# springmeyer/cov-tiles

Hardware: AMD Instinct MI355X
Metric: GB/s raw COVT bytes decoded + Mvertices/s, z2–z14 tile batch, 1/2/4/8 GPU (higher is better)
Workload: dtype int32

## Files before the change

cov-tiles_amd/__init__.py:

```python
from __future__ import annotations

import ctypes as C
import os
import subprocess
from dataclasses import dataclass
from typing import List, NamedTuple, Optional

import numpy as np

_HERE = os.path.dirname(os.path.abspath(__file__))
_LIB = os.path.join(_HERE, os.environ.get("COVT_LIB_VARIANT", "libcovt.so"))

OK = 0
ERR_UNSUPPORTED_ENCODING = -1
ERR_TRUNCATED = -2
ERR_COUNT_MISMATCH = -3
ERR_BAD_HEADER = -4
ERR_DEVICE = -5
ERR_INVALID_ARG = -6
INPUT_PADDING = 4096
FORMAT_GENC, FORMAT_GEND = 0, 1
FAMILY_RLE, FAMILY_VARINT, FAMILY_FASTPFOR, FAMILY_LANE, FAMILY_SPLIT, FAMILY_SPLIT_FPF, FAMILY_SPLIT_RLE = range(7)
NUM_FAMILIES = 7
DESC_LANE, DESC_SPLIT, DESC_SPLIT_PAD, DESC_SPLIT_FPF = 0x1, 0x2, 0x4, 0x8
# ... 1142 lines not shown

    def feature(self, i: int) -> bytes:
        if not 0 <= i < len(self):
            raise IndexError(i)
        return bytes(self.data[int(self.offsets[i]):int(self.offsets[i + 1])])


@dataclass
class BboxColumn:
    xmin: np.ndarray
    ymin: np.ndarray
    xmax: np.ndarray
    ymax: np.ndarray
    extent: np.ndarray
    n_empty: int = 0

    def __len__(self) -> int:
        return int(self.xmin.size)

    def as_struct(self) -> np.ndarray:
        return np.stack([self.xmin, self.ymin, self.xmax, self.ymax], axis=1)


@dataclass
class MeasuresColumn:
    area: np.ndarray
    length: np.ndarray
    num_coords: np.ndarray

    def __len__(self) -> int:
        return int(self.area.size)


@dataclass
class PropertyColumn:
    name: str
    type: int
    n_features: int
    validity: np.ndarray
    values: np.ndarray
    dict_offsets: Optional[np.ndarray]
    dict_bytes: Optional[np.ndarray]
    n_valid: int

    def valid(self, i: int) -> bool:
        return bool((int(self.validity[i >> 3]) >> (i & 7)) & 1)

    def value(self, i: int):
        if not self.valid(i):
            return None
        if self.type == PROP_BOOLEAN:
            return bool((int(self.values[i >> 3]) >> (i & 7)) & 1)
        if self.type == PROP_INT64:
            return int(self.values[i])
        if self.type == PROP_FLOAT:
            return float(self.values[i])
        k = int(self.values[i])
        return bytes(self.dict_bytes[self.dict_offsets[k]:self.dict_offsets[k + 1]]).decode("utf-8")

    def to_list(self):
        return [self.value(i) for i in range(self.n_features)]


@dataclass
class LayerColumns:
    layer: int
    ids: Optional[np.ndarray]
    geometry: GeometryColumn
    num_bits: int = 0
    column_type: int = 0
    properties: Optional[dict] = None
    wkb: Optional[WkbColumn] = None
    bbox: Optional[BboxColumn] = None
    crs: int = CRS_TILE
    measures: Optional["MeasuresColumn"] = None


_GEOM_FIELD = {GEOMETRY_TYPES: "geometryTypes", GEOMETRY_OFFSETS: "geometryOffsets", PART_OFFSETS: "partOffsets",
               RING_OFFSETS: "ringOffsets", VERTEX_OFFSETS: "vertexOffsets", VERTEX_BUFFER: "vertexBuffer"}


def split_layers(plan: Plan, out: np.ndarray, res: np.ndarray, tile: int = 0) -> List[LayerColumns]:
    layers = {}
    for i in np.nonzero(plan.streams["tile"] == tile)[0]:
        s = plan.streams[i]
        _raise(int(res[i][0]), "stream %d (layer %d, type %d)" % (i, s["layer"], s["stream_type"]))
        if int(s["column_kind"]) == 2:
            continue
        lc = layers.setdefault(int(s["layer"]), LayerColumns(int(s["layer"]), None, GeometryColumn()))
        arr = plan.stream_array(out, int(i))
        if int(s["column_kind"]) == 0:
            lc.ids = arr
        else:
            setattr(lc.geometry, _GEOM_FIELD[int(s["stream_type"])], arr)
            lc.num_bits = int(s["num_bits"])
            lc.column_type = int(s["column_type"])
    return [layers[k] for k in sorted(layers)]


class CovtParser:
    @staticmethod
    def decode_covt(covt_buffer: bytes, fmt: int = FORMAT_GENC, id_mode: int = ID_FORMAT,
                    properties: bool = False, tile_id=None, crs: int = CRS_TILE) -> List[LayerColumns]:
        if crs != CRS_TILE and tile_id is None:
            raise IllegalArgumentException("a CRS other than CRS_TILE needs the tile's (z, x, y)")
        geo = (crs, [tile_id]) if crs != CRS_TILE else (None, None)
        plan = Plan.from_tiles([covt_buffer], fmt, id_mode, PLAN_PROPERTIES if properties else 0)
        _raise(int(plan.tile_status[0]), "decodeLayerMetadata")
        out, res = plan.decode_host()
        layers = split_layers(plan, out, res, 0)
        for lc in layers:
            lc.crs = crs
        if plan.num_geometry_columns:
            wbuf, wres = plan.wkb_host(*geo)
            by_layer = {lc.layer: lc for lc in layers}
            for c in range(plan.num_geometry_columns):
                lc = by_layer.get(int(plan.wkb["layer"][c]))
                if lc is not None and int(wres["status"][c]) == OK:
                    lc.wkb = plan.wkb_column(wbuf, wres, c)
            bbuf, bres = plan.bbox_host(*geo)
            for c in range(plan.num_geometry_columns):
                lc = by_layer.get(int(plan.bbox["layer"][c]))
                if lc is not None and int(bres["status"][c]) == OK:
                    lc.bbox = plan.bbox_column(bbuf, bres, c)
            mbuf, mres = plan.measures_host()
            for c in range(plan.num_geometry_columns):
                lc = by_layer.get(int(plan.measures["layer"][c]))
                if lc is not None and int(mres["status"][c]) == OK:
                    lc.measures = plan.measures_column(mbuf, mres, c)
        if properties and plan.num_property_columns:
            buf, pres = plan.properties_host()
            by_layer = {lc.layer: lc for lc in layers}
            for c in range(plan.num_property_columns):
                L = int(plan.props["layer"][c])
                lc = by_layer.setdefault(L, LayerColumns(L, None, GeometryColumn()))
                if lc.properties is None:
                    lc.properties = {}
                col = plan.property_column(buf, pres, c)
                lc.properties[col.name] = col
            layers = [by_layer[k] for k in sorted(by_layer)]
        return layers


def version() -> str:
    return lib().covt_version().decode()


_BUILD_SOURCES = (
    ("csrc/covt_decode.hip", "csrc/covt_assemble.hip", "csrc/covt_props.hip", "csrc/covt_plan_device.hip",
     "csrc/covt_wkb.hip", "csrc/covt_bbox.hip", "csrc/covt_measures.hip", "csrc/covt_host.cpp")
    + ("../include/covt.h", "csrc/covt_internal.h", "csrc/covt_wave.h", "csrc/covt_segscan.h", "csrc/covt_walk.h",
       "csrc/covt_props_plan.h",
       "csrc/covt_scratch.h", "csrc/covt_coop.h", "csrc/covt_wkb_plan.h", "csrc/covt_bbox_plan.h",
       "csrc/covt_measures_plan.h", "csrc/covt_geo_plan.h", "csrc/covt_arena.h", "csrc/covt_split_plan.h"))


def source_build_id() -> str:
    import hashlib

    h = hashlib.sha256()
    for f in _BUILD_SOURCES:
        with open(os.path.join(_HERE, f), "rb") as fh:
            h.update(fh.read())
    return h.hexdigest()[:16]


def library_build_id() -> str:
    v = version()
    return v.rsplit("src:", 1)[1] if "src:" in v else "unknown"
```

cov-tiles_amd/csrc/covt_decode.hip:

```cpp
#include <hip/hip_runtime.h>
#include <stdint.h>

#include "covt.h"
#include "covt_internal.h"
#include "covt_wave.h"
#include "covt_walk.h"

namespace covt {

constexpr int kWin = 1024;

#ifndef COVT_LONG_STREAM
#define COVT_LONG_STREAM 16384
#endif
#ifndef COVT_LONG_PRIO
#define COVT_LONG_PRIO 2
#endif
#ifndef COVT_RLE_SHORT_SPAN
#define COVT_RLE_SHORT_SPAN 448
#endif
#ifndef COVT_CHUNK_PRIO
#define COVT_CHUNK_PRIO 2
#endif
constexpr int kLongStream = COVT_LONG_STREAM;
#ifdef COVT_TIMING
constexpr int kPhases = 8;
__device__ uint32_t* covt_phase_buf;
__device__ const covt_stream_desc* covt_phase_desc0;
#endif

typedef __attribute__((address_space(3))) const uint16_t lds_cu16;

struct __attribute__((aligned(16))) WaveSmem {
    int32_t misc[4];
    uint16_t cpre[64];
    uint16_t cmask[64];
    union alignas(16) {
        struct {
            uint32_t win[kWin / 4 + 4];
            uint16_t list[kWin];
            uint16_t next[kWin + 8];
            uint16_t grec[64];
        } v;
        struct {
            union {
                uint32_t stage[324];
                uint32_t ring[512];
            };
            uint32_t patch[256];
            uint32_t cbuf[260];
            union {
                uint8_t posx[2][192];
                uint32_t xw[224];
            };
        } f;
    } u;
};
constexpr int kSmemHdr = 272;
constexpr int kFamSmemRle = kSmemHdr + (kWin / 4 + 4) * 4 + kWin * 2 + (kWin + 8) * 2 + 64 * 2;
constexpr int kFamSmemVarint = kSmemHdr + (kWin / 4 + 4) * 4 + kWin * 2;
constexpr int kFamSmemFpf = kSmemHdr + (512 + 256 + 260 + 224) * 4 > kFamSmemVarint
                                ? kSmemHdr + (512 + 256 + 260 + 224) * 4
                                : kFamSmemVarint;
constexpr int kFpfXw = 224;
static_assert(kFamSmemFpf >= kSmemHdr + (int)sizeof(((WaveSmem*)nullptr)->u.f), "FastPFOR scratch stride");
static_assert(kFamSmemVarint >= kSmemHdr + (int)sizeof(((WaveSmem*)nullptr)->u.v.win) +
                                    (int)sizeof(((WaveSmem*)nullptr)->u.v.list), "varint scratch stride");
static_assert(__builtin_offsetof(WaveSmem, u) == kSmemHdr, "WaveSmem header size");
static_assert(kFamSmemRle == (int)sizeof(WaveSmem), "RLE uses the whole scratch");
static_assert(kFamSmemRle % 16 == 0 && kFamSmemVarint % 16 == 0 && kFamSmemFpf % 16 == 0, "16-B strides");

typedef uint32_t u32x4 __attribute__((ext_vector_type(4)));
typedef __attribute__((address_space(1))) const uint32_t g_u32;
typedef __attribute__((address_space(1))) const u32x4 g_v4;
__device__ __forceinline__ const g_u32* g32(uintptr_t a) { return (const g_u32*)a; }
__device__ __forceinline__ uint4 ld128(uintptr_t a16) {
    const u32x4 v = *(const g_v4*)a16;
    return make_uint4(v.x, v.y, v.z, v.w);
}
typedef __attribute__((address_space(1))) const uint8_t g_u8;
__device__ __forceinline__ uint4 ld128_off(const g_u8* base, uint32_t off) {
    const u32x4 v = *(const g_v4*)(base + off);
    return make_uint4(v.x, v.y, v.z, v.w);
}

__device__ __forceinline__ uint32_t ld_le32(const uint8_t* p) {
    const uintptr_t a = (uintptr_t)p;
    const g_u32* q = g32(a & ~(uintptr_t)3);
    return __builtin_amdgcn_alignbyte(q[1], q[0], (uint32_t)(a & 3));
}
__device__ __forceinline__ uint32_t ld_be32(const uint8_t* p) { return __builtin_bswap32(ld_le32(p)); }
__host__ __device__ constexpr uint32_t be_sel(uint32_t sh) {
    return (sh + 3u) | ((sh + 2u) << 8) | ((sh + 1u) << 16) | (sh << 24);
}
__device__ __forceinline__ uint32_t be_word(uint32_t hi, uint32_t lo, uint32_t sel) {
    return __builtin_amdgcn_perm(hi, lo, sel);
}
typedef __attribute__((address_space(4))) const uint32_t c_u32;
typedef __attribute__((address_space(4))) const u32x4 c_v4;
__device__ __forceinline__ uint32_t sld_le32(const uint8_t* p) {
    const uintptr_t a = (uintptr_t)p;
    const c_u32* q = (const c_u32*)(a & ~(uintptr_t)3);
    const uint64_t v = ((uint64_t)q[1] << 32) | q[0];
    return (uint32_t)(v >> (8u * (uint32_t)(a & 3u)));
}
__device__ __forceinline__ uint32_t sld_be32(const uint8_t* p) { return uniu(__builtin_bswap32(sld_le32(p))); }
__device__ __forceinline__ uint4 sld128(uintptr_t a16) {
    const u32x4 v = *(const c_v4*)a16;
    return make_uint4(v.x, v.y, v.z, v.w);
}

__device__ __forceinline__ uint32_t hibits4(uint32_t x) {
    x &= 0x80808080u;
    return ((x >> 7) & 1u) | ((x >> 14) & 2u) | ((x >> 21) & 4u) | ((x >> 28) & 8u);
}
__device__ __forceinline__ uint32_t hibits16(uint4 d) {
    return hibits4(d.x) | (hibits4(d.y) << 4) | (hibits4(d.z) << 8) | (hibits4(d.w) << 12);
}
__device__ __forceinline__ uint32_t range16(int32_t s, int32_t e) {
    s = s < 0 ? 0 : (s > 16 ? 16 : s);
    e = e < 0 ? 0 : (e > 16 ? 16 : e);
    if (e <= s) return 0u;
    return ((1u << e) - 1u) & ~((1u << s) - 1u);
}
typedef unsigned short u16x2 __attribute__((ext_vector_type(2)));
__device__ __forceinline__ uint32_t pext7(uint32_t x) {
    x &= 0x7f7f7f7fu;
    const uint32_t y = __builtin_bit_cast(uint32_t, __builtin_bit_cast(u16x2, x) >> (u16x2){1, 1});
    const uint32_t t = (x & 0x007f007fu) | (y & ~0x007f007fu);
    return (t & 0x3fffu) | ((t >> 2) & ~0x3fffu);
}
__device__ __forceinline__ uint32_t bytemask(int n) {
    return n >= 4 ? 0xffffffffu : (n <= 0 ? 0u : ((1u << (8 * n)) - 1u));
}
__device__ __forceinline__ int32_t zz32(uint32_t e) { return (int32_t)((e >> 1) ^ (0u - (e & 1u))); }
__device__ __forceinline__ int64_t zz64(uint64_t e) { return (int64_t)((e >> 1) ^ (0ull - (e & 1ull))); }

__host__ __device__ __forceinline__ void morton_xy(int32_t code, int nb, uint32_t& x, uint32_t& y) {
    uint32_t v = (uint32_t)code, t;
    t = (v ^ (v >> 1)) & 0x22222222u; v ^= t ^ (t << 1);
    t = (v ^ (v >> 2)) & 0x0c0c0c0cu; v ^= t ^ (t << 2);
    t = (v ^ (v >> 4)) & 0x00f000f0u; v ^= t ^ (t << 4);
    t = (v ^ (v >> 8)) & 0x0000ff00u; v ^= t ^ (t << 8);
    const uint32_t low = nb >= 16 ? 0xffffu : (nb <= 0 ? 0u : ((1u << nb) - 1u));
    const uint32_t top = nb <= 16 ? 0u : ((nb >= 32 ? 0xffffffffu : ((1u << nb) - 1u)) & ~0xffffu);
    const uint32_t hi = code < 0 ? top : 0u;
    x = (v & low) | hi;
    y = ((v >> 16) & low) | hi;
}
__device__ __forceinline__ int32_t morton_half(int nb) {
    const int32_t te = (int32_t)(2u << ((uint32_t)(nb - 2) & 31u));
    return te / 2;
}

struct Carry {
    uint32_t x, y;
};

typedef int32_t i32x4 __attribute__((ext_vector_type(4)));
// ... 1276 lines not shown
            COVT_PHASE(c, 0);
            const int32_t nblocks_page = uni(thissize / kFpfBlock);
            const int32_t jb0 = v0 > done ? min((v0 - done) / kFpfBlock, nblocks_page) : 0;
            const int32_t nblocks = v1 <= done ? 0 : uni(min(nblocks_page, (int32_t)(((int64_t)v1 - done + kFpfBlock - 1) / kFpfBlock)));
            const int32_t nw32 = (int32_t)nw;
            const int32_t bclen = uni((int32_t)(bcw * 4));
            const uint8_t* cb8 = (const uint8_t*)sm.u.f.cbuf;
            int32_t cbase = (int32_t)(4 * (mw0 - bc));
            auto chunk_load = [&](int32_t at) {
                cbase = (int32_t)(4 * (load_words(sm.u.f.cbuf, bc + (at >> 2)) - bc));
            };
            auto walk = [&](int32_t cur, FpfHdr& h) -> int32_t {
                cur = uni(cur);
                cbase = uni(cbase);
                if (!xin && (uint32_t)(cur - cbase) > (uint32_t)(1020 - 260)) chunk_load(cur);
                const int32_t j = cur - cbase;
                const uint32_t hw =
                    uniu(__builtin_amdgcn_alignbyte(sm.u.f.cbuf[(j >> 2) + 1], sm.u.f.cbuf[j >> 2], (uint32_t)j & 3u));
                const int32_t b = (int32_t)(int8_t)(hw & 0xffu);
                const int32_t ce = (int32_t)((hw >> 8) & 0xffu);
                const int32_t hasx = ce > 0 ? 1 : 0;
                const int32_t idx = hasx ? (int32_t)(int8_t)((hw >> 16) & 0xffu) - b : 1;
                const int32_t k = (uint32_t)(idx - 2) <= 30u ? idx : 0;
                const int32_t xsz = __builtin_amdgcn_readlane(xz_v, k);
                const int32_t xc = __builtin_amdgcn_readlane(xc_v, k);
                h.b = b;
                h.ce = ce;
                h.idx = idx;
                h.xcur = (uint32_t)xc;
                h.bcoff = cur + 2 + hasx;
                h.next = h.bcoff + ce;
                xc_v += l == k ? ce : 0;
                const int32_t worst = max(max(max(b - 32, -b), h.next - bclen), max(max(idx - 32, 1 - idx), xc + ce - xsz));
                return worst > 0 ? COVT_ERR_BAD_HEADER : COVT_OK;
            };
            auto xword = [&](int32_t k, uint32_t xs, uint32_t i, uint32_t& xbit) -> int32_t {
                const uint32_t bit = __umul24(i & 31u, (uint32_t)k);
                xbit = bit & 31u;
                return (int32_t)(xs + __umul24(i >> 5, (uint32_t)k) + (bit >> 5));
            };
            auto prefetch = [&](const FpfHdr& hv, int32_t pkv, FpfPre& pr, int slot, bool raw = true) {
                FpfHdr h;
                h.idx = uni(hv.idx);
                h.ce = uni(hv.ce);
                h.xcur = uniu(hv.xcur);
                h.bcoff = uni(hv.bcoff);
                const int32_t pk = uni(pkv);
                if (raw) {
                    const uintptr_t a16 = ((uintptr_t)c.sb + 4u * (uint32_t)pk) & ~(uintptr_t)15;
                    const uint32_t lraw = min((uint32_t)l, 2u * (uint32_t)uni(hv.b) + 1u);
                    pr.raw = ld128_off((const g_u8*)a16, 16u * lraw);
                }
                const int32_t k = h.idx;
                const uint32_t xs = k >= 2 ? (uint32_t)__builtin_amdgcn_readlane(xs_v, k) : 0u;
                uint32_t xb;
                const int32_t wx = xword(k >= 2 ? k : 2, xs, h.xcur + (uint32_t)l, xb);
                const uint32_t xon = (uint32_t)(k >= 2) & (uint32_t)(l < h.ce) & (uint32_t)(wx < nw32);
                if (!xin) {
                    const uint32_t wi = (uint32_t)wx & (0u - xon);
                    const u32x3 xv = *(const g_v3*)((const g_u8*)(((uintptr_t)c.sb) & ~(uintptr_t)3) + 4u * wi);
                    pr.x0 = xv.x;
                    pr.x1 = xv.y;
                    pr.x2 = xv.z;
                }
                const int32_t pb = h.bcoff - cbase;
                pr.pos = cb8[min(pb + l, 4 * 260 - 1)];
                if (h.ce > 64) {
#pragma unroll
                    for (int q = 1; q < 4; ++q)
                        sm.u.f.posx[slot][64 * (q - 1) + l] = cb8[min(pb + l + 64 * q, 4 * 260 - 1)];
                }
            };
            FpfHdr h;
            int32_t pk = (int32_t)p0 + 1;
            int32_t cur0 = 0;
            if (jb0 > 0 && jb0 < nblocks && !c.err) {
                if (skip && skip->done == done) {
                    cur0 = skip->cur0;
                    pk = skip->pk;
                    xc_v = skip->xc;
                } else {
                    int32_t cur = 0, pkk = pk;
                    for (int32_t j = 0; j < jb0; ++j) {
                        if (!xin && (uint32_t)(cur - cbase) > (uint32_t)(1020 - 8)) chunk_load(cur);
                        const int32_t jj = cur - cbase;
                        const uint32_t hw = uniu(__builtin_amdgcn_alignbyte(sm.u.f.cbuf[(jj >> 2) + 1],
                                                                            sm.u.f.cbuf[jj >> 2], (uint32_t)jj & 3u));
                        const int32_t b = (int32_t)(int8_t)(hw & 0xffu);
                        const int32_t ce = (int32_t)((hw >> 8) & 0xffu);
                        const int32_t idx = (int32_t)(int8_t)((hw >> 16) & 0xffu) - b;
                        pkk += 8 * b;
                        xc_v += (ce > 0 && idx >= 2 && idx <= 32 && l == idx) ? ce : 0;
                        cur += ce > 0 ? 3 + ce : 2;
                        if (cur > bclen) { c.err = COVT_ERR_BAD_HEADER; break; }
                    }
                    cur0 = uni(cur);
                    pk = uni(pkk);
                    if (skip) {
                        skip->done = done;
                        skip->cur0 = cur0;
                        skip->pk = pk;
                        skip->xc = xc_v;
                    }
                }
                COVT_PHASE(c, 0);
            }
            auto block = [&](int32_t j, const FpfPre& pc, FpfPre& pn, int slot) {
                FpfHdr hc;
                hc.b = uni(h.b);
                hc.ce = uni(h.ce);
                hc.idx = uni(h.idx);
                hc.xcur = uniu(h.xcur);
                hc.bcoff = uni(h.bcoff);
                hc.next = uni(h.next);
                const int32_t pkc = uni(pk);
                const int32_t b = hc.b;
                const uint32_t o = (sbmis + 4u * (uint32_t)pkc) & 15u;
                const int32_t qoff = (int32_t)(o >> 2);
                {
                    uint4 raw2 = make_uint4(0, 0, 0, 0);
                    if (b == 32) {
                        const uintptr_t a16 = ((uintptr_t)c.sb + 4u * (uint32_t)pkc) & ~(uintptr_t)15;
                        raw2 = sld128(a16 + 1024);
                    }
                    const uint32_t nxt = lane_next(pc.raw.x, raw2.x);
                    uint4 wv;
                    wv.x = be_word(pc.raw.y, pc.raw.x, bsel);
                    wv.y = be_word(pc.raw.z, pc.raw.y, bsel);
                    wv.z = be_word(pc.raw.w, pc.raw.z, bsel);
                    wv.w = be_word(nxt, pc.raw.w, bsel);
                    ((uint4*)sm.u.f.stage)[l] = wv;
                    if (b == 32 && l == 0) {
                        uint4 w2;
                        w2.x = be_word(raw2.y, raw2.x, bsel);
                        w2.y = be_word(raw2.z, raw2.y, bsel);
                        w2.z = be_word(raw2.w, raw2.z, bsel);
                        w2.w = be_word(0u, raw2.w, bsel);
                        ((uint4*)sm.u.f.stage)[64] = w2;
                    }
                }
                if (hc.ce > 0) ((uint4*)sm.u.f.patch)[l] = make_uint4(0, 0, 0, 0);
                wave_sync();
                COVT_PHASE(c, 1);
                if (j + 1 < nblocks) {
                    c.err = walk(hc.next, h);
                    pk = pkc + 8 * b;
                    if (!c.err && pk + 8 * h.b > nw32) c.err = COVT_ERR_TRUNCATED;
                    if (c.err) return;
                }
                prefetch(h, pk, pn, slot ^ 1);
                COVT_PHASE(c, 2);
                uint32_t v[4];
                {
                    const uint32_t mask = b == 32 ? 0xffffffffu : ((1u << b) - 1u);
                    uint32_t bit = __umul24((uint32_t)(l & 7) * 4u, (uint32_t)b);
                    const int32_t wb = (int32_t)__umul24((uint32_t)(l >> 3), (uint32_t)b) + qoff;
#pragma unroll
                    for (int k = 0; k < 4; ++k) {
                        const int32_t wi = wb + (int32_t)(bit >> 5);
                        const uint32_t lo = sm.u.f.stage[wi], hi = sm.u.f.stage[wi + 1];
                        v[k] = __builtin_amdgcn_alignbit(hi, lo, bit & 31u) & mask;
                        bit += (uint32_t)b;
                    }
                }
                COVT_PHASE(c, 3);
#if defined(COVT_ABL_NOEXC)
                if (false) {
#else
                if (hc.ce > 0) {
#endif
                    const int32_t k = hc.idx;
                    const uint32_t xs = k >= 2 ? (uint32_t)__builtin_amdgcn_readlane(xs_v, k) : 0u;
                    const bool el = l < hc.ce;
                    uint32_t ex = 1u;
                    if (k != 1) {
                        uint32_t xbit;
                        const int32_t wi = xword(k, xs, hc.xcur + (uint32_t)l, xbit);
                        uint32_t lo, hi;
                        if (xin) {
                            const int32_t m = el ? wi - (int32_t)mw0 : 0;
                            lo = sm.u.f.cbuf[m];
                            hi = sm.u.f.cbuf[m + 1];
                        } else {
                            lo = wi < nw32 ? be_word(pc.x1, pc.x0, bsel) : 0u;
                            hi = wi + 1 < nw32 ? be_word(pc.x2, pc.x1, bsel) : 0u;
                        }
                        const uint32_t m = k == 32 ? 0xffffffffu : ((1u << k) - 1u);
                        ex = __builtin_amdgcn_alignbit(hi, lo, xbit) & m;
                    }
                    atomicOr(&sm.u.f.patch[el ? pc.pos : (uint32_t)(4 * l)], el ? ex << (b & 31) : 0u);
                    if (hc.ce > 64) {
                        for (int q = 1; q < 4; ++q) {
                            const int32_t e = l + 64 * q;
                            if (e < hc.ce) {
                                const uint32_t ex = k == 1 ? 1u : xget(W, xs, k, hc.xcur + (uint32_t)e);
                                atomicOr(&sm.u.f.patch[sm.u.f.posx[slot][64 * (q - 1) + l]], ex << (b & 31));
                            }
                        }
                    }
                    wave_sync();
                    const uint4 pt = ((const uint4*)sm.u.f.patch)[l];
                    v[0] |= pt.x;
                    v[1] |= pt.y;
                    v[2] |= pt.z;
                    v[3] |= pt.w;
                }
                COVT_PHASE(c, 4);
#if defined(COVT_ABL_NOSTORE)
                sink_values<OP, 4>(v, 0, 0, kFpfBlock, c.nb, c.out, cr);
#else
                if (sum_only)
                    sum_values<OP, 4>(v, (int64_t)done + (int64_t)j * kFpfBlock, kFpfBlock, ax, ay);
                else
                    sink_values<OP, 4>(v, (int64_t)done + (int64_t)j * kFpfBlock, 0, kFpfBlock, c.nb, c.out, cr);
#endif
                wave_sync();
                COVT_PHASE(c, 5);
            };
            FpfPre preB;
            if (jb0 < nblocks && !c.err) {
                c.err = walk(cur0, h);
                if (!c.err && pk + 8 * h.b > nw32) c.err = COVT_ERR_TRUNCATED;
                if (!c.err) {
                    prefetch(h, pk, pre, 0, !spec);
                    if (!sum_only) fpf_prime_stores<OP>(c.out, (int64_t)done + (int64_t)jb0 * kFpfBlock);
                    int32_t j = jb0;
                    do {
                        block(j, pre, preB, 0);
                        if (j + 1 < nblocks && !c.err) block(j + 1, preB, pre, 1);
                        j += 2;
                    } while (j < nblocks && !c.err);
                }
            }
            done += thissize;
            p = ie;
            if (done >= v1) break;
        }
        decoded = L;
        if (!c.err && has_end && p < nw) {
            int32_t vpos = (int32_t)(4 * p);
            const int32_t base = L;
            Win w;
            w.valid = false;
            const bool tail_in = L > 0 && ((int64_t)(vpos & ~15) >> 2) >= mw0 && nw - mw0 <= 255;
            const int32_t got = varint_take<MODE_WORDREV, VAL_VB>(
                sm, c.sb, w, vpos, (int32_t)(4 * nw), c.n - L, true, c.err,
                [&](const uint32_t (&lo)[1], const uint32_t (&hi)[1], int32_t vb, int32_t, int32_t count) {
                    if (sum_only) sum_values<OP, 1>(lo, (int64_t)base + vb, count, ax, ay);
                    else sink_values<OP, 1>(lo, (int64_t)base + vb, 0, count, c.nb, c.out, cr);
                },
                0, nullptr, 0, tail_in ? sm.u.f.cbuf : nullptr, (int32_t)mw0);
            decoded = L + got;
        }
    }
    if (!c.err && has_end) {
        for (int32_t b = decoded; !sum_only && b < c.n; b += 64) {
            uint32_t vv[1] = {0};
            sink_values<OP, 1>(vv, b, 0, c.n - b < 64 ? c.n - b : 64, c.nb, c.out, cr);
        }
        if (OP == COVT_OP_FPF_ZZ_DELTA_XY && (c.n & 1)) c.err = COVT_ERR_COUNT_MISMATCH;
    }
    COVT_PHASE(c, 7);
    c.consumed = c.byte_length;
    if (sum_only) {
        sums->x = lane_bcast(incl_scan(ax), 63);
        sums->y = lane_bcast(incl_scan(ay), 63);
    }
    if (fin) *fin = cr;
}

template <int OP>
__device__ __forceinline__ void run_fastpfor_stream(Ctx& c) {
    WaveSmem& sm = *c.sm;
    const int l = lane_id();
    const Words W{c.sb, c.byte_length / 4};
    const int32_t nw32 = W.nw;
    const uint32_t bsel = be_sel((uint32_t)((uintptr_t)c.sb & 3u));
    Carry cr{0u, 0u};
    int32_t decoded = 0;
    int32_t L = 0;
    int32_t p = 1;
    int xs_v = 0, xz_v = -1, xc_v = 0;
    int32_t mw0 = 0;
    if (c.byte_length > c.avail) { c.err = COVT_ERR_TRUNCATED; }
    if (!c.err && nw32 > 0) {
        const uint32_t head0 = W.uniform(0), head1 = W.uniform(1);
        L = (int32_t)head0;
        if (L < 0) c.err = COVT_ERR_BAD_HEADER;
        L -= L % kFpfBlock;
        if (!c.err && L > c.n) c.err = COVT_ERR_COUNT_MISMATCH;
        int32_t done = 0;
        const uintptr_t s_end = (uintptr_t)c.sb + 4u * (uint32_t)nw32;
        struct WordsRaw {
            uint4 r;
            int32_t base;
            uint32_t sh;
        };
        auto words_issue = [&](int32_t w) -> WordsRaw {
            const uintptr_t addr = (uintptr_t)c.sb + 4u * (uint32_t)w;
            const uintptr_t a16 = addr & ~(uintptr_t)15;
            const uint32_t o = (uint32_t)(addr & 15u);
            const uint32_t lmax = s_end > a16 ? (uint32_t)((s_end - 1 - a16) >> 4) : 0u;
            WordsRaw q;
            q.r = ld128_off((const g_u8*)a16, 16u * min((uint32_t)l, lmax));
            q.base = uni(w - (int32_t)(o >> 2));
            q.sh = o & 3u;
            return q;
        };
        auto words_store = [&](uint32_t* dst, const WordsRaw& q) -> int32_t {
            const uint32_t nx = lane_next(q.r.x);
            const uint32_t sel = be_sel(q.sh);
            const int32_t wl = q.base + 4 * l;
            uint4 wv;
            wv.x = wl < nw32 ? be_word(q.r.y, q.r.x, sel) : 0u;
            wv.y = wl + 1 < nw32 ? be_word(q.r.z, q.r.y, sel) : 0u;
            wv.z = wl + 2 < nw32 ? be_word(q.r.w, q.r.z, sel) : 0u;
            wv.w = wl + 3 < nw32 ? be_word(nx, q.r.w, sel) : 0u;
            wave_sync();
            ((uint4*)dst)[l] = wv;
            wave_sync();
            return q.base;
        };
        auto load_words = [&](uint32_t* dst, int32_t w) -> int32_t { return words_store(dst, words_issue(w)); };
        while (!c.err && done < L) {
            done = uni(done);
            const int32_t thissize = uni((L - done) < kFpfPage ? (L - done) : kFpfPage);
            const int32_t p0 = uni(p);
            if (p0 >= nw32) { c.err = COVT_ERR_TRUNCATED; break; }
            const int64_t ie0 = (int64_t)p0 + (int32_t)(p0 == 1 ? head1 : W.uniform(p0));
            if (ie0 < 0 || ie0 >= nw32) { c.err = COVT_ERR_TRUNCATED; break; }
            int32_t ie = (int32_t)ie0;
            const WordsRaw mq = words_issue(ie);
            const uintptr_t pa = (uintptr_t)c.sb + 4u * (uint32_t)(p0 + 1);
            const uintptr_t A0 = pa & ~(uintptr_t)127;
            const uint32_t glast = s_end > A0 ? (uint32_t)((s_end - 1 - A0) & ~(uintptr_t)15) : 0u;
            const int32_t wbase = uni((int32_t)(p0 + 1) - (int32_t)((pa - A0) >> 2));
            uint4 R = ld128_off((const g_u8*)A0, min(16u * (uint32_t)l, glast));
            int32_t kst = 0;
            int32_t vend = wbase;
            uint32_t prev63 = 0u;
            mw0 = words_store(sm.u.f.cbuf, mq);
            auto mword = [&](int32_t w) -> uint32_t { return uniu(sm.u.f.cbuf[w - mw0]); };
            const int32_t bytesize = (int32_t)mword(ie++);
            if (bytesize < 0 || bytesize > kFpfBcCap) { c.err = COVT_ERR_BAD_HEADER; break; }
            xc_v = 0;
            const int32_t bcw = (bytesize + 3) / 4;
            const int32_t bc = ie;
            if (bc + bcw >= nw32) { c.err = COVT_ERR_TRUNCATED; break; }
            ie += bcw;
            int64_t ie64 = ie;
            {
                int32_t dbase = INT32_MIN / 2;
                auto dword = [&](int32_t w) -> uint32_t {
                    if (w >= mw0 && w < mw0 + 255) return mword(w);
                    if (w < dbase || w >= dbase + 255) dbase = load_words(sm.u.f.ring, w);
                    return uniu(sm.u.f.ring[w - dbase]);
                };
                uint32_t bm = dword((int32_t)ie64++) & ~1u;
                xs_v = 0;
                xz_v = -1;
                while (bm) {
                    const int32_t k = __builtin_ctz(bm) + 1;
                    bm &= bm - 1;
                    if (ie64 >= nw32) { c.err = COVT_ERR_TRUNCATED; break; }
                    const int32_t size = (int32_t)dword((int32_t)ie64++);
                    if (size < 0) { c.err = COVT_ERR_BAD_HEADER; break; }
                    const int64_t groups = ((int64_t)size + 31) / 32;
                    xs_v = l == k ? (int)(uint32_t)ie64 : xs_v;
                    xz_v = l == k ? size : xz_v;
                    ie64 += groups * k;
                    ie64 -= ((groups * 32 - size) * k) / 32;
                }
                if (c.err) break;
            }
            const bool xin = ie64 - mw0 <= 255;
            ie = (int32_t)(ie64 < nw32 ? ie64 : (int64_t)nw32);
            COVT_PHASE(c, 0);
            const int32_t nblocks = uni(thissize / kFpfBlock);
            const int32_t bclen = uni((int32_t)(bcw * 4));
            const uint8_t* cb8 = (const uint8_t*)sm.u.f.cbuf;
            const g_u8* cbyte = (const g_u8*)(c.sb + 4u * (uint32_t)bc);
            int32_t cbase = (int32_t)(4 * (mw0 - bc));
            auto chunk_load = [&](int32_t at) {
                cbase = (int32_t)(4 * (load_words(sm.u.f.cbuf, bc + (at >> 2)) - bc));
            };
            bool fin = false;
            int32_t bneed = INT32_MAX;
            auto stage = [&]() {
                const int32_t k = uni(kst);
                const uint32_t nx = lane_next(R.x, 0u);
                const int32_t w0 = wbase + 256 * k + 4 * l;
                uint4 wv;
                wv.x = w0 < nw32 ? be_word(R.y, R.x, bsel) : 0u;
                wv.y = w0 + 1 < nw32 ? be_word(R.z, R.y, bsel) : 0u;
                wv.z = w0 + 2 < nw32 ? be_word(R.w, R.z, bsel) : 0u;
                wv.w = w0 + 3 < nw32 ? be_word(nx, R.w, bsel) : 0u;
                const int32_t fw = wbase + 256 * k - 1;
                const uint32_t fix = fw < nw32 ? be_word(lane_bcast(R.x, 0), prev63, bsel) : 0u;
                prev63 = lane_bcast(R.w, 63);
                const uint32_t ri = (uint32_t)(256 * k + 4 * l) & 511u;
                wave_sync();
                if (l < 63) {
                    *(uint4*)&sm.u.f.ring[ri] = wv;
                } else {
                    sm.u.f.ring[ri] = wv.x;
                    sm.u.f.ring[ri + 1] = wv.y;
                    sm.u.f.ring[ri + 2] = wv.z;
                }
                if (l == 0 && k > 0) sm.u.f.ring[(uint32_t)(256 * k - 1) & 511u] = fix;
                wave_sync();
                kst = k + 1;
                vend = wbase + 256 * (k + 1) - 1;
                if (!fin || vend < bneed)
                    R = ld128_off((const g_u8*)A0, min(1024u * (uint32_t)(k + 1) + 16u * (uint32_t)l, glast));
                wave_sync();
            };
            int32_t cur = 0, pk = (int32_t)p0 + 1;
            for (int32_t jbat = 0, nbat = 0; jbat < nblocks && !c.err; jbat += nbat) {
                jbat = uni(jbat);
                nbat = uni(min(64, nblocks - jbat));
                uint32_t hw_v = 0u;
                int32_t cur_v = bclen + 1;
                cur = uni(cur);
                cbase = uni(cbase);
                if (!xin && cur <= bclen && (uint32_t)(cur - cbase) > (uint32_t)(1020 - 258)) chunk_load(cur);
                for (int32_t g = 0; g < nbat; ++g) {
                    cur = uni(cur);
                    cbase = uni(cbase);
                    if (cur > bclen) break;
                    if (!xin && cur - cbase > 1020 - 8) {
                        nbat = g;
                        break;
                    }
                    const int32_t q = cur - cbase;
                    const uint32_t hw =
                        uniu(__builtin_amdgcn_alignbyte(sm.u.f.cbuf[(q >> 2) + 1], sm.u.f.cbuf[q >> 2], (uint32_t)q & 3u));
                    const int32_t ce = (int32_t)((hw >> 8) & 0xffu);
                    const int32_t nx = cur + (ce > 0 ? 3 + ce : 2);
                    if (!xin && g > 0 && nx - cbase > 1020) {
                        nbat = g;
                        break;
                    }
                    hw_v = l == g ? hw : hw_v;
                    cur_v = l == g ? cur : cur_v;
                    cur = nx;
                }
                nbat = uni(nbat);
                if (nbat == 0) {
                    c.err = COVT_ERR_BAD_HEADER;
                    break;
                }
                COVT_PHASE(c, 1);
                const bool in = l < nbat;
                const int32_t b_v = (int32_t)(int8_t)(hw_v & 0xffu);
                const int32_t ce_v = (int32_t)((hw_v >> 8) & 0xffu);
                const bool hasx = ce_v > 0;
                const int32_t idx_v = hasx ? (int32_t)(int8_t)((hw_v >> 16) & 0xffu) - b_v : 1;
                const bool arr_k = hasx && idx_v >= 2 && idx_v <= 32;
                const bool arr = in && arr_k;
                int32_t xcur_v = 0;
                for (uint64_t todo = __ballot(arr); todo;) {
                    const int32_t kk = __builtin_amdgcn_readlane(idx_v, (int32_t)__builtin_ctzll(todo));
                    const bool mine = arr && idx_v == kk;
                    const uint32_t v = mine ? (uint32_t)ce_v : 0u;
                    const uint32_t s = incl_scan(v);
                    const int32_t base = __builtin_amdgcn_readlane(xc_v, kk);
                    xcur_v = mine ? base + (int32_t)(s - v) : xcur_v;
                    xc_v += l == kk ? (int32_t)lane_bcast(s, 63) : 0;
                    todo &= ~__ballot(mine);
                }
                const uint32_t w8 = in ? 8u * (uint32_t)(b_v & 63) : 0u;
                const uint32_t pinc = incl_scan(w8);
                const int32_t pk_v = pk + (int32_t)(pinc - w8);
                pk += (int32_t)lane_bcast(pinc, 63);
                int32_t nok = nbat;
                int32_t ferr = 0;
                {
                    const int32_t xsz = lane_get(xz_v, arr_k ? idx_v : 0);
                    bool bad = (uint32_t)b_v > 32u || cur_v + 2 > bclen;
                    bad |= hasx && (cur_v + 3 + ce_v > bclen || (idx_v != 1 && !arr_k));
                    bad |= arr_k && (xsz < 0 || xcur_v + ce_v > xsz);
                    const bool trunc = pk_v + 8 * b_v > nw32;
                    const uint64_t fail = __ballot(in && (bad || trunc));
                    if (fail) {
                        nok = (int32_t)__builtin_ctzll(fail);
                        ferr = __builtin_amdgcn_readlane(bad ? COVT_ERR_BAD_HEADER : COVT_ERR_TRUNCATED, nok);
                    }
                }
                COVT_PHASE(c, 2);
                fin = jbat + nbat >= nblocks || ferr != 0;
                bneed = nok > 0 ? uni(__builtin_amdgcn_readlane(pk_v + 8 * b_v, nok - 1)) : 0;
                if (jbat == 0) stage();
                struct Hdr {
                    int32_t b, ce, idx, pk, bcoff, xo;
                    uint32_t xcur;
                };
                int32_t xo_v = 255;
                if (!xin) {
                    const bool ab = arr && l < nok;
                    const int32_t k = ab ? idx_v : 2;
                    const uint32_t xs = (uint32_t)lane_get(xs_v, k);
                    const uint32_t b0 = __umul24((uint32_t)xcur_v, (uint32_t)k);
                    const uint32_t b1 = __umul24((uint32_t)(xcur_v + ce_v), (uint32_t)k);
                    const int32_t wlo = (int32_t)(xs + (b0 >> 5));
                    const int32_t wn = ab ? (int32_t)((b1 + 31u) >> 5) - (int32_t)(b0 >> 5) + 1 : 0;
                    const uint32_t winc = incl_scan((uint32_t)wn);
                    const int32_t wo = (int32_t)(winc - (uint32_t)wn);
                    const int32_t wend = (int32_t)winc;
                    xo_v = ab && wend <= kFpfXw ? wo : 255;
                    const int32_t tot = uni(min((int32_t)lane_bcast(winc, 63), kFpfXw));
                    const g_u8* sb4 = (const g_u8*)(((uintptr_t)c.sb) & ~(uintptr_t)3);
                    u32x2 d[4];
                    bool okw[4];
#pragma unroll
                    for (int r = 0; r < 4; ++r) {
                        const int32_t t = 64 * r + l;
                        int32_t lo = 0, hi = 64;
#pragma unroll
                        for (int s2 = 0; s2 < 7; ++s2) {
                            const int32_t mid = (lo + hi) >> 1;
                            const bool le = lane_get(wend, mid & 63) <= t;
                            const bool act = lo < hi;
                            lo = act && le ? mid + 1 : lo;
                            hi = act && !le ? mid : hi;
                        }
                        const int32_t g = min(lo, 63);
                        const int32_t w = lane_get(wlo, g) + (t - lane_get(wo, g));
                        okw[r] = t < tot && w < nw32;
                        d[r] = *(const g_v2*)(sb4 + 4u * (okw[r] ? (uint32_t)w : 0u));
                    }
#pragma unroll
                    for (int r = 0; r < 4; ++r)
                        if (64 * r + l < kFpfXw) sm.u.f.xw[64 * r + l] = okw[r] ? be_word(d[r].y, d[r].x, bsel) : 0u;
                    wave_sync();
                }
                const uint32_t f_v = (uint32_t)(b_v & 0xff) | ((uint32_t)ce_v << 8) | ((uint32_t)(idx_v & 0xff) << 16) |
                                     ((uint32_t)xo_v << 24);
                const int32_t bo_v = cur_v + (hasx ? 3 : 2);
                auto rec = [&](int32_t g, Hdr& h) {
                    const uint32_t f = uniu((uint32_t)__builtin_amdgcn_readlane((int32_t)f_v, g));
                    h.b = (int32_t)(f & 0xffu);
                    h.ce = (int32_t)((f >> 8) & 0xffu);
                    h.idx = (int32_t)(int8_t)((f >> 16) & 0xffu);
                    h.xo = (int32_t)(f >> 24);
                    h.xcur = uniu((uint32_t)__builtin_amdgcn_readlane(xcur_v, g));
                    h.bcoff = uni(__builtin_amdgcn_readlane(bo_v, g));
                    h.pk = uni(__builtin_amdgcn_readlane(pk_v, g));
                };
                fpf_prime_stores<OP>(c.out, (int64_t)done + (int64_t)jbat * kFpfBlock);
                auto block = [&](int32_t g) {
                    Hdr hc;
                    rec(g, hc);
                    const int32_t b = hc.b;
                    if (uni(vend) < hc.pk + 8 * b) stage();
                    if (hc.ce > 0) ((uint4*)sm.u.f.patch)[l] = make_uint4(0, 0, 0, 0);
                    COVT_PHASE(c, 3);
                    uint32_t v[4];
                    {
                        const uint32_t mask = b == 32 ? 0xffffffffu : ((1u << b) - 1u);
                        uint32_t bit = __umul24((uint32_t)(l & 7) * 4u, (uint32_t)b);
                        const int32_t r0 = (hc.pk - wbase) & 511;
                        const int32_t wb = (int32_t)__umul24((uint32_t)(l >> 3), (uint32_t)b) + r0;
                        if (r0 + 8 * b <= 511) {
#pragma unroll
                            for (int k = 0; k < 4; ++k) {
                                const int32_t wi = wb + (int32_t)(bit >> 5);
                                const uint32_t lo = sm.u.f.ring[wi], hi = sm.u.f.ring[wi + 1];
                                v[k] = __builtin_amdgcn_alignbit(hi, lo, bit & 31u) & mask;
                                bit += (uint32_t)b;
                            }
                        } else {
#pragma unroll
                            for (int k = 0; k < 4; ++k) {
                                const int32_t wi = wb + (int32_t)(bit >> 5);
                                const uint32_t lo = sm.u.f.ring[wi & 511], hi = sm.u.f.ring[(wi + 1) & 511];
                                v[k] = __builtin_amdgcn_alignbit(hi, lo, bit & 31u) & mask;
                                bit += (uint32_t)b;
                            }
                        }
                    }
                    COVT_PHASE(c, 4);
                    if (hc.ce > 0) {
                        const int32_t k = hc.idx;
                        const bool el = l < hc.ce;
                        const uint32_t pos = cb8[min(max(hc.bcoff - cbase + l, 0), 4 * 260 - 1)];
                        uint32_t ex = 1u;
                        if (k != 1) {
                            const uint32_t xs = (uint32_t)__builtin_amdgcn_readlane(xs_v, k);
                            const uint32_t bb = __umul24(hc.xcur + (uint32_t)l, (uint32_t)k);
                            const uint32_t xbit = bb & 31u;
                            uint32_t lo, hi;
                            if (xin) {
                                const int32_t m = el ? (int32_t)(xs + (bb >> 5)) - mw0 : 0;
                                lo = sm.u.f.cbuf[m];
                                hi = sm.u.f.cbuf[m + 1];
                            } else if (hc.xo != 255) {
                                const int32_t m = el ? hc.xo + (int32_t)(bb >> 5) - (int32_t)(__umul24(hc.xcur, (uint32_t)k) >> 5) : 0;
                                lo = sm.u.f.xw[m];
                                hi = sm.u.f.xw[m + 1];
                            } else {
                                const int32_t wi = (int32_t)(xs + (bb >> 5));
                                lo = el && wi < nw32 ? W(wi) : 0u;
                                hi = el && wi + 1 < nw32 ? W(wi + 1) : 0u;
                            }
                            const uint32_t m = k == 32 ? 0xffffffffu : ((1u << k) - 1u);
                            ex = __builtin_amdgcn_alignbit(hi, lo, xbit) & m;
                        }
                        atomicOr(&sm.u.f.patch[el ? pos : (uint32_t)(4 * l)], el ? ex << (b & 31) : 0u);
                        if (hc.ce > 64) {
                            const uint32_t xs = k >= 2 ? (uint32_t)__builtin_amdgcn_readlane(xs_v, k) : 0u;
                            for (int q = 1; q < 4; ++q) {
                                const int32_t e = l + 64 * q;
                                if (e < hc.ce) {
                                    const uint32_t ex2 = k == 1 ? 1u : xget(W, xs, k, hc.xcur + (uint32_t)e);
                                    const uint32_t ps = cbyte[(hc.bcoff + e) ^ 3];
                                    atomicOr(&sm.u.f.patch[ps], ex2 << (b & 31));
                                }
                            }
                        }
                        wave_sync();
                        const uint4 pt = ((const uint4*)sm.u.f.patch)[l];
                        v[0] |= pt.x;
                        v[1] |= pt.y;
                        v[2] |= pt.z;
                        v[3] |= pt.w;
                    }
                    COVT_PHASE(c, 5);
                    sink_values<OP, 4>(v, (int64_t)done + (int64_t)(jbat + g) * kFpfBlock, 0, kFpfBlock, c.nb, c.out, cr);
                    wave_sync();
                    COVT_PHASE(c, 6);
                };
                for (int32_t g = 0; g < nok; ++g) {
                    g = uni(g);
                    block(g);
                }
                if (ferr) c.err = ferr;
            }
            done += thissize;
            p = ie;
        }
        decoded = L;
        if (!c.err && p < nw32) {
            int32_t vpos = (int32_t)(4 * p);
            const int32_t base = L;
            Win w;
            w.valid = false;
            const bool tail_in = L > 0 && ((vpos & ~15) >> 2) >= mw0 && nw32 - mw0 <= 255;
            const int32_t got = varint_take<MODE_WORDREV, VAL_VB>(
                sm, c.sb, w, vpos, 4 * nw32, c.n - L, true, c.err,
                [&](const uint32_t (&lo)[1], const uint32_t (&hi)[1], int32_t vb, int32_t, int32_t count) {
                    sink_values<OP, 1>(lo, (int64_t)base + vb, 0, count, c.nb, c.out, cr);
                },
                0, nullptr, 0, tail_in ? sm.u.f.cbuf : nullptr, (int32_t)mw0);
            decoded = L + got;
        }
    }
    if (!c.err) {
        for (int32_t b = decoded; b < c.n; b += 64) {
            uint32_t vv[1] = {0};
            sink_values<OP, 1>(vv, b, 0, c.n - b < 64 ? c.n - b : 64, c.nb, c.out, cr);
        }
        if (OP == COVT_OP_FPF_ZZ_DELTA_XY && (c.n & 1)) c.err = COVT_ERR_COUNT_MISMATCH;
    }
    COVT_PHASE(c, 7);
    c.consumed = c.byte_length;
}

template <int OP>
__device__ __forceinline__ void fpf_add_carry(uint8_t* out, int32_t v0, int32_t v1, Carry cr) {
    const uint32_t cx = cr.x, cy = OP == COVT_OP_FPF_ZZ_DELTA_XY ? cr.y : cr.x;
    if ((cx | cy) == 0u) return;
    __builtin_amdgcn_s_waitcnt(0x0f70);
    int32_t* o = (int32_t*)out;
    typedef __attribute__((address_space(1))) i32x4 g_i4;
    const int32_t nq = (v1 - v0) >> 2;
    const int32_t last = v0 + 4 * (nq > 0 ? nq - 1 : 0);
    constexpr int kDeep = 8;
    for (int32_t q0 = 0; q0 < nq; q0 += 64 * kDeep) {
        i32x4 v[kDeep];
#pragma unroll
        for (int k = 0; k < kDeep; ++k) v[k] = *(const g_i4*)(o + min(v0 + 4 * (q0 + 64 * k + lane_id()), last));
#pragma unroll
        for (int k = 0; k < kDeep; ++k) {
            const int32_t q = q0 + 64 * k + lane_id();
            if (q < nq)
                st_out16(o + v0 + 4 * q, make_int4((int32_t)((uint32_t)v[k].x + cx), (int32_t)((uint32_t)v[k].y + cy),
                                                   (int32_t)((uint32_t)v[k].z + cx), (int32_t)((uint32_t)v[k].w + cy)));
        }
    }
    const int32_t i = v0 + 4 * nq + lane_id();
    if (i < v1) o[i] = (int32_t)((uint32_t)o[i] + (((i - v0) & 1) ? cy : cx));
}

constexpr int kSplitSlots = COVT_SPLIT_SLOTS;
struct Agg {
    int32_t cnt;
    uint32_t sx, sy;
};
__device__ __forceinline__ Agg agg_cat(const Agg& a, const Agg& b, bool xy) {
    if (a.cnt < 0) return a;
    if (b.cnt < 0) return Agg{b.cnt, b.sx, (uint32_t)a.cnt + b.sy};
    const bool sw = xy && (a.cnt & 1);
    return Agg{a.cnt + b.cnt, a.sx + (sw ? b.sy : b.sx), a.sy + (sw ? b.sx : b.sy)};
}
typedef __attribute__((address_space(1))) uint64_t g_u64;
__device__ __forceinline__ void rec_publish(covt_stream_result* rec, const Agg& a, uint32_t tag) {
    if (lane_id() == 0) {
        g_u64* g = (g_u64*)rec;
        const uint64_t t = (uint64_t)tag << 32;
        __hip_atomic_store(g, t | (uint32_t)a.cnt, __ATOMIC_RELAXED, __HIP_MEMORY_SCOPE_AGENT);
        __hip_atomic_store(g + 1, t | a.sx, __ATOMIC_RELAXED, __HIP_MEMORY_SCOPE_AGENT);
        __hip_atomic_store(g + 2, t | a.sy, __ATOMIC_RELAXED, __HIP_MEMORY_SCOPE_AGENT);
    }
}
__device__ __forceinline__ bool rec_try(covt_stream_result* rec, uint32_t tag, Agg& a) {
    g_u64* g = (g_u64*)rec;
    const uint64_t x0 = __hip_atomic_load(g, __ATOMIC_RELAXED, __HIP_MEMORY_SCOPE_AGENT);
    const uint64_t x1 = __hip_atomic_load(g + 1, __ATOMIC_RELAXED, __HIP_MEMORY_SCOPE_AGENT);
    const uint64_t x2 = __hip_atomic_load(g + 2, __ATOMIC_RELAXED, __HIP_MEMORY_SCOPE_AGENT);
    const bool ok = (uint32_t)(x0 >> 32) == tag && (uint32_t)(x1 >> 32) == tag && (uint32_t)(x2 >> 32) == tag;
    a = Agg{(int32_t)(uint32_t)x0, (uint32_t)x1, (uint32_t)x2};
    return uniu(ok ? 1u : 0u) != 0u;
}
constexpr int kRecAgg = 1, kRecIncl = 4, kRecTicket = 7;
static_assert(kSplitSlots == 8, "split record layout");
constexpr uint32_t kSpinLimit = 1u << 22;
__device__ Agg lookback(covt_stream_result* res, int64_t t, int32_t chunk, bool xy, int32_t& err) {
    Agg acc{0, 0u, 0u};
    int64_t k = t - 1;
    uint32_t spins = 0;
    for (int32_t left = chunk; left > 0;) {
        covt_stream_result* r = res + kSplitSlots * k;
        Agg a;
        if (rec_try(r + kRecIncl, 2u, a)) {
            acc = agg_cat(a, acc, xy);
            break;
        }
        if (rec_try(r + kRecAgg, 1u, a)) {
            acc = agg_cat(a, acc, xy);
            --k;
            --left;
            continue;
        }
        if (++spins > kSpinLimit) { err = COVT_ERR_DEVICE; break; }
        __builtin_amdgcn_s_sleep(2);
    }
    return acc;
}

template <int OP>
__device__ __forceinline__ void run_varint_chunk(Ctx& c, int32_t s, int32_t e, int32_t chunk, covt_stream_result* res, int64_t t) {
    constexpr bool kU64 = OP == COVT_OP_VARINT_U64 || OP == COVT_OP_VARINT_ZZ_S64;
    constexpr int kVal = kU64 ? VAL_U64_STRICT : VAL_J4;
    constexpr bool kXY = OP == COVT_OP_VARINT_ZZ_DELTA_XY;
    constexpr bool kZZ = OP == COVT_OP_VARINT_ZZ_I32 || OP == COVT_OP_VARINT_ZZ_DELTA_I32 || kXY ||
                         OP == COVT_OP_VARINT_ZZ_I32_AS_I64 || OP == COVT_OP_VARINT_ZZ_DELTA_I64;
    constexpr bool kSum = OP == COVT_OP_VARINT_ZZ_DELTA_I32 || kXY || OP == COVT_OP_VARINT_DELTA_MORTON ||
                          OP == COVT_OP_VARINT_ZZ_DELTA_I64;
    const int l = lane_id();
    int32_t p = 0;
    if (chunk > 0) {
        const uintptr_t lo = (uintptr_t)c.sb & ~(uintptr_t)15;
        int32_t hi = s, last = -1;
        while (hi > 0) {
            uintptr_t w0 = ((uintptr_t)(c.sb + hi) & ~(uintptr_t)15);
            w0 = w0 >= lo + 1008 ? w0 - 1008 : lo;
            const uint4 d = ld128(w0 + 16 * (uintptr_t)l);
            const int32_t q0 = (int32_t)((intptr_t)(w0 + 16 * (uintptr_t)l) - (intptr_t)c.sb);
            const uint32_t T = ~hibits16(d) & 0xffffu & range16(-q0, hi - q0);
            const uint32_t best = T ? (uint32_t)(q0 + 31 - __builtin_clz(T)) + 1u : 0u;
            const uint32_t m = wave_max(best);
// ... 827 lines not shown
```

Measured before the change: 654.1.

## Specialize FastPFor bit-unpack by width and simplify exception patch loop

Adds a shared fpf_unpack4 helper that, for bit widths up to 8 or 16, loads two or three LDS words once and extracts the four values with bitfield-extract instead of doing eight LDS reads and four funnel shifts per lane. Both the short-stream and ring-buffer paths use it; the ring path now always masks indices, dropping the separate unwrapped fast path. The exception patch loop becomes one uniform loop over 64-lane groups that reads positions from the LDS chunk buffer rather than global bytes. The binary search over block ends is bounded by the live block count instead of a fixed seven steps. Costs are more branching on b and dynamic loop trip counts.

```diff
diff --git a/cov-tiles_amd/__init__.py b/cov-tiles_amd/__init__.py
--- a/cov-tiles_amd/__init__.py
+++ b/cov-tiles_amd/__init__.py
@@ -1318,7 +1318,8 @@
     + ("../include/covt.h", "csrc/covt_internal.h", "csrc/covt_wave.h", "csrc/covt_segscan.h", "csrc/covt_walk.h",
        "csrc/covt_props_plan.h",
        "csrc/covt_scratch.h", "csrc/covt_coop.h", "csrc/covt_wkb_plan.h", "csrc/covt_bbox_plan.h",
-       "csrc/covt_measures_plan.h", "csrc/covt_geo_plan.h", "csrc/covt_arena.h", "csrc/covt_split_plan.h"))
+       "csrc/covt_measures_plan.h", "csrc/covt_geo_plan.h", "csrc/covt_arena.h", "csrc/covt_split_plan.h",
+       "csrc/covt_fpf_unpack.h"))
 
 
 def source_build_id() -> str:
diff --git a/cov-tiles_amd/csrc/covt_decode.hip b/cov-tiles_amd/csrc/covt_decode.hip
--- a/cov-tiles_amd/csrc/covt_decode.hip
+++ b/cov-tiles_amd/csrc/covt_decode.hip
@@ -5,6 +5,7 @@
 #include "covt_internal.h"
 #include "covt_wave.h"
 #include "covt_walk.h"
+#include "covt_fpf_unpack.h"
 
 namespace covt {
 
@@ -1587,16 +1588,8 @@
                 COVT_PHASE(c, 2);
                 uint32_t v[4];
                 {
-                    const uint32_t mask = b == 32 ? 0xffffffffu : ((1u << b) - 1u);
-                    uint32_t bit = __umul24((uint32_t)(l & 7) * 4u, (uint32_t)b);
-                    const int32_t wb = (int32_t)__umul24((uint32_t)(l >> 3), (uint32_t)b) + qoff;
-#pragma unroll
-                    for (int k = 0; k < 4; ++k) {
-                        const int32_t wi = wb + (int32_t)(bit >> 5);
-                        const uint32_t lo = sm.u.f.stage[wi], hi = sm.u.f.stage[wi + 1];
-                        v[k] = __builtin_amdgcn_alignbit(hi, lo, bit & 31u) & mask;
-                        bit += (uint32_t)b;
-                    }
+                    const uint32_t* stg = sm.u.f.stage;
+                    fpf_unpack4([&](int32_t i) { return stg[i]; }, qoff, b, l, v);
                 }
                 COVT_PHASE(c, 3);
 #if defined(COVT_ABL_NOEXC)
@@ -1814,7 +1807,6 @@
             const int32_t nblocks = uni(thissize / kFpfBlock);
             const int32_t bclen = uni((int32_t)(bcw * 4));
             const uint8_t* cb8 = (const uint8_t*)sm.u.f.cbuf;
-            const g_u8* cbyte = (const g_u8*)(c.sb + 4u * (uint32_t)bc);
             int32_t cbase = (int32_t)(4 * (mw0 - bc));
             auto chunk_load = [&](int32_t at) {
                 cbase = (int32_t)(4 * (load_words(sm.u.f.cbuf, bc + (at >> 2)) - bc));
@@ -1947,12 +1939,15 @@
                     const g_u8* sb4 = (const g_u8*)(((uintptr_t)c.sb) & ~(uintptr_t)3);
                     u32x2 d[4];
                     bool okw[4];
+                    const int32_t nstep = uni(32 - __builtin_clz((uint32_t)nok | 1u));
 #pragma unroll
                     for (int r = 0; r < 4; ++r) {
+                        okw[r] = false;
+                        d[r] = u32x2{0u, 0u};
+                        if (64 * r >= tot) continue;
                         const int32_t t = 64 * r + l;
-                        int32_t lo = 0, hi = 64;
-#pragma unroll
-                        for (int s2 = 0; s2 < 7; ++s2) {
+                        int32_t lo = 0, hi = nok;
+                        for (int32_t s2 = 0; s2 < nstep; ++s2) {
                             const int32_t mid = (lo + hi) >> 1;
                             const bool le = lane_get(wend, mid & 63) <= t;
                             const bool act = lo < hi;
@@ -1992,66 +1987,40 @@
                     COVT_PHASE(c, 3);
                     uint32_t v[4];
                     {
-                        const uint32_t mask = b == 32 ? 0xffffffffu : ((1u << b) - 1u);
-                        uint32_t bit = __umul24((uint32_t)(l & 7) * 4u, (uint32_t)b);
                         const int32_t r0 = (hc.pk - wbase) & 511;
-                        const int32_t wb = (int32_t)__umul24((uint32_t)(l >> 3), (uint32_t)b) + r0;
-                        if (r0 + 8 * b <= 511) {
-#pragma unroll
-                            for (int k = 0; k < 4; ++k) {
-                                const int32_t wi = wb + (int32_t)(bit >> 5);
-                                const uint32_t lo = sm.u.f.ring[wi], hi = sm.u.f.ring[wi + 1];
-                                v[k] = __builtin_amdgcn_alignbit(hi, lo, bit & 31u) & mask;
-                                bit += (uint32_t)b;
-                            }
-                        } else {
-#pragma unroll
-                            for (int k = 0; k < 4; ++k) {
-                                const int32_t wi = wb + (int32_t)(bit >> 5);
-                                const uint32_t lo = sm.u.f.ring[wi & 511], hi = sm.u.f.ring[(wi + 1) & 511];
-                                v[k] = __builtin_amdgcn_alignbit(hi, lo, bit & 31u) & mask;
-                                bit += (uint32_t)b;
-                            }
-                        }
+                        const uint32_t* ring = sm.u.f.ring;
+                        fpf_unpack4([&](int32_t i) { return ring[i & 511]; }, r0, b, l, v);
                     }
                     COVT_PHASE(c, 4);
                     if (hc.ce > 0) {
                         const int32_t k = hc.idx;
-                        const bool el = l < hc.ce;
-                        const uint32_t pos = cb8[min(max(hc.bcoff - cbase + l, 0), 4 * 260 - 1)];
-                        uint32_t ex = 1u;
-                        if (k != 1) {
-                            const uint32_t xs = (uint32_t)__builtin_amdgcn_readlane(xs_v, k);
-                            const uint32_t bb = __umul24(hc.xcur + (uint32_t)l, (uint32_t)k);
-                            const uint32_t xbit = bb & 31u;
-                            uint32_t lo, hi;
-                            if (xin) {
-                                const int32_t m = el ? (int32_t)(xs + (bb >> 5)) - mw0 : 0;
-                                lo = sm.u.f.cbuf[m];
-                                hi = sm.u.f.cbuf[m + 1];
-                            } else if (hc.xo != 255) {
-                                const int32_t m = el ? hc.xo + (int32_t)(bb >> 5) - (int32_t)(__umul24(hc.xcur, (uint32_t)k) >> 5) : 0;
-                                lo = sm.u.f.xw[m];
-                                hi = sm.u.f.xw[m + 1];
-                            } else {
-                                const int32_t wi = (int32_t)(xs + (bb >> 5));
-                                lo = el && wi < nw32 ? W(wi) : 0u;
-                                hi = el && wi + 1 < nw32 ? W(wi + 1) : 0u;
+                        for (int32_t e0 = 0; e0 < hc.ce; e0 += 64) {
+                            const int32_t e = e0 + l;
+                            const bool el = e < hc.ce;
+                            const uint32_t pos = cb8[min(max(hc.bcoff - cbase + e, 0), 4 * 260 - 1)];
+                            uint32_t ex = 1u;
+                            if (k != 1) {
+                                const uint32_t xs = (uint32_t)__builtin_amdgcn_readlane(xs_v, k);
+                                const uint32_t bb = __umul24(hc.xcur + (uint32_t)e, (uint32_t)k);
+                                const uint32_t xbit = bb & 31u;
+                                uint32_t lo, hi;
+                                if (xin) {
+                                    const int32_t m = el ? (int32_t)(xs + (bb >> 5)) - mw0 : 0;
+                                    lo = sm.u.f.cbuf[m];
+                                    hi = sm.u.f.cbuf[m + 1];
+                                } else if (hc.xo != 255) {
+                                    const int32_t m = el ? hc.xo + (int32_t)(bb >> 5) - (int32_t)(__umul24(hc.xcur, (uint32_t)k) >> 5) : 0;
+                                    lo = sm.u.f.xw[m];
+                                    hi = sm.u.f.xw[m + 1];
+                                } else {
+                                    const int32_t wi = (int32_t)(xs + (bb >> 5));
+                                    lo = el && wi < nw32 ? W(wi) : 0u;
+                                    hi = el && wi + 1 < nw32 ? W(wi + 1) : 0u;
+                                }
+                                const uint32_t m = k == 32 ? 0xffffffffu : ((1u << k) - 1u);
+                                ex = __builtin_amdgcn_alignbit(hi, lo, xbit) & m;
                             }
-                            const uint32_t m = k == 32 ? 0xffffffffu : ((1u << k) - 1u);
-                            ex = __builtin_amdgcn_alignbit(hi, lo, xbit) & m;
-                        }
-                        atomicOr(&sm.u.f.patch[el ? pos : (uint32_t)(4 * l)], el ? ex << (b & 31) : 0u);
-                        if (hc.ce > 64) {
-                            const uint32_t xs = k >= 2 ? (uint32_t)__builtin_amdgcn_readlane(xs_v, k) : 0u;
-                            for (int q = 1; q < 4; ++q) {
-                                const int32_t e = l + 64 * q;
-                                if (e < hc.ce) {
-                                    const uint32_t ex2 = k == 1 ? 1u : xget(W, xs, k, hc.xcur + (uint32_t)e);
-                                    const uint32_t ps = cbyte[(hc.bcoff + e) ^ 3];
-                                    atomicOr(&sm.u.f.patch[ps], ex2 << (b & 31));
-                                }
-                            }
+                            atomicOr(&sm.u.f.patch[el ? pos : (uint32_t)(4 * l)], el ? ex << (b & 31) : 0u);
                         }
                         wave_sync();
                         const uint4 pt = ((const uint4*)sm.u.f.patch)[l];
diff --git a/cov-tiles_amd/csrc/covt_fpf_unpack.h b/cov-tiles_amd/csrc/covt_fpf_unpack.h
--- /dev/null
+++ b/cov-tiles_amd/csrc/covt_fpf_unpack.h
@@ -0,0 +1,59 @@
+#pragma once
+#include <stdint.h>
+
+#if defined(__HIPCC__) || defined(__CUDACC__)
+#define COVT_FPF_HD __host__ __device__
+#else
+#define COVT_FPF_HD
+#endif
+
+COVT_FPF_HD inline uint32_t fpf_funnel(uint32_t hi, uint32_t lo, uint32_t sh) {
+#if defined(__HIP_DEVICE_COMPILE__)
+    return __builtin_amdgcn_alignbit(hi, lo, sh);
+#else
+    return (uint32_t)(((((uint64_t)hi) << 32) | lo) >> (sh & 31u));
+#endif
+}
+COVT_FPF_HD inline uint32_t fpf_field(uint32_t x, uint32_t off, uint32_t width) {
+#if defined(__HIP_DEVICE_COMPILE__)
+    return __builtin_amdgcn_ubfe(x, off, width);
+#else
+    return (x >> off) & (width >= 32u ? 0xffffffffu : ((1u << width) - 1u));
+#endif
+}
+
+template <class WordFn>
+COVT_FPF_HD inline void fpf_unpack4(WordFn word, int32_t r0, int32_t b, int lane, uint32_t (&v)[4]) {
+    if (b == 0) {
+        v[0] = v[1] = v[2] = v[3] = 0u;
+        return;
+    }
+    const uint32_t ub = (uint32_t)b;
+    const uint32_t bit0 = (uint32_t)(lane & 7) * 4u * ub;
+    const int32_t wb = r0 + (int32_t)((uint32_t)(lane >> 3) * ub);
+    if (b <= 8) {
+        const int32_t w = wb + (int32_t)(bit0 >> 5);
+        const uint32_t s = fpf_funnel(word(w + 1), word(w), bit0 & 31u);
+        v[0] = fpf_field(s, 0u, ub);
+        v[1] = fpf_field(s, ub, ub);
+        v[2] = fpf_field(s, 2u * ub, ub);
+        v[3] = fpf_field(s, 3u * ub, ub);
+    } else if (b <= 16) {
+        const int32_t w = wb + (int32_t)(bit0 >> 5);
+        const uint32_t w0 = word(w), w1 = word(w + 1), w2 = word(w + 2);
+        const uint32_t lo = fpf_funnel(w1, w0, bit0 & 31u), hi = fpf_funnel(w2, w1, bit0 & 31u);
+        const uint32_t mid = b == 16 ? hi : fpf_funnel(hi, lo, 2u * ub);
+        v[0] = fpf_field(lo, 0u, ub);
+        v[1] = fpf_field(lo, ub, ub);
+        v[2] = fpf_field(mid, 0u, ub);
+        v[3] = fpf_field(mid, ub, ub);
+    } else {
+        const uint32_t mask = b == 32 ? 0xffffffffu : ((1u << ub) - 1u);
+        uint32_t bit = bit0;
+        for (int k = 0; k < 4; ++k) {
+            const int32_t w = wb + (int32_t)(bit >> 5);
+            v[k] = fpf_funnel(word(w + 1), word(w), bit & 31u) & mask;
+            bit += ub;
+        }
+    }
+}
```

Measured after the change: 644.8. -1.4%, worse.
